# travistangvh/time-series-kafka-demo

Hardware: AMD Instinct MI355X
Metric: waveform_windows_per_sec (higher is better)
Workload: dtype bf16; 1 GPU; model=MyCNN5, global_batch=65536, seq_len=120, streams_per_gpu=65536, fs_hz=125, hipgraph=True, overlap=False, parallelism=dp1, mode=pipeline

## Files before the change

### tskd_amd/ops/csrc/preprocess_kernels.hip

```cpp

#include <hip/hip_runtime.h>
#include <cstdlib>
#include <math.h>

#include "tskd_common.h"

typedef __attribute__((ext_vector_type(4))) unsigned int u32x4_;
typedef __attribute__((ext_vector_type(4))) float f32x4_;

__device__ __forceinline__ long ring_head(const long long* dstate, long h) {
    return dstate ? (long)dstate[0] : h;
}
__device__ __forceinline__ long ring_nproc(const long long* dstate, long p) {
    return dstate ? (long)dstate[1] : p;
}

__global__ void advance_state_kernel(long long* dstate, int nb, int np) {
    if (threadIdx.x == 0 && blockIdx.x == 0) {
        dstate[0] += nb;
        dstate[1] += np;
    }
}

typedef float f32x2p_ __attribute__((ext_vector_type(2)));

#define ING_GRP 4
#define ING_GL 16
template <class DT>
__global__ void ingest_dense_kernel(
    const DT* __restrict__ raw,
    float* __restrict__ bsum,
    float* __restrict__ bcnt,
    const int* __restrict__ chan_map,
    int S, int CIN, int C, int T, int G,
    int bucket_len, long head_in,
    const long long* __restrict__ dstate, int BST)
{
    const long head = ring_head(dstate, head_in);
    const int head_mod = (int)(head % G);
    const int NB = T / bucket_len;
    const int NBG = (NB + ING_GRP - 1) / ING_GRP;
    const long nwaves = (long)S * CIN * NBG;
    const int wlane = threadIdx.x % WAVE;
    const int grp = wlane / ING_GL;
    const int lane = wlane % ING_GL;
    for (long w = (long)blockIdx.x * (blockDim.x / WAVE) + threadIdx.x / WAVE;
         w < nwaves; w += (long)gridDim.x * (blockDim.x / WAVE)) {
        const int wi = (int)w;
        const int bg = wi % NBG;
        const int wrem = wi / NBG;
        const int cin = wrem % CIN;
        const int s = wrem / CIN;
        const int b = bg * ING_GRP + grp;
        const bool active = b < NB;
        const DT* src = raw + ((long)s * CIN + cin) * T +
                        (long)(active ? b : 0) * bucket_len;
        float sum = 0.f, cnt = 0.f;
        if (active) {
            if constexpr (sizeof(DT) == 2) {
                const unsigned short* su = (const unsigned short*)src;
                const int mis = (int)(((size_t)su & 15) / 2);
                const u32x4_* vp = (const u32x4_*)(su - mis);
                const bool at_end = s == S - 1 && cin == CIN - 1 &&
                                    b == NB - 1;
                const int nch = (mis + bucket_len + (at_end ? 0 : 7)) / 8;
                for (int base = lane; base < nch; base += 5 * ING_GL) {
                    union { u32x4_ q; unsigned short h[8]; } v[5];
                    #pragma unroll
                    for (int u = 0; u < 5; ++u) {
                        const int pp = base + u * ING_GL;
                        v[u].q = __builtin_nontemporal_load(
                            &vp[pp < nch ? pp : 0]);
                    }
                    #pragma unroll
                    for (int u = 0; u < 5; ++u) {
                        const int pp = base + u * ING_GL;
                        if (pp >= nch) continue;
                        const int idx0 = pp * 8 - mis;
                        if (idx0 >= 0 && idx0 + 8 <= bucket_len) {
                            #pragma unroll
                            for (int j = 0; j < 8; ++j) {
                                const float f = bf16_to_f32(v[u].h[j]);
                                if (!isnan(f)) { sum += f; cnt += 1.f; }
                            }
                        } else {
                            #pragma unroll
                            for (int j = 0; j < 8; ++j) {
                                const unsigned k = (unsigned)(idx0 + j);
                                if (k < (unsigned)bucket_len) {
                                    const float f = bf16_to_f32(v[u].h[j]);
                                    if (!isnan(f)) { sum += f; cnt += 1.f; }
                                }
                            }
                        }
                    }
                }
                if (at_end)
                    for (int i = nch * 8 - mis + lane; i < bucket_len;
                         i += ING_GL) {
                        const float f = bf16_to_f32(su[i]);
                        if (!isnan(f)) { sum += f; cnt += 1.f; }
                    }
            } else {
                int pre = (int)(((16 - ((size_t)src & 15)) & 15) / 4);
                if (pre > bucket_len) pre = bucket_len;
                for (int i = lane; i < pre; i += ING_GL) {
                    const float f = (float)src[i];
                    if (!isnan(f)) { sum += f; cnt += 1.f; }
                }
                const int quad = (bucket_len - pre) / 4;
                const f32x4_* vp = (const f32x4_*)((const float*)src + pre);
                for (int base = lane; base < quad; base += 5 * ING_GL) {
                    f32x4_ v[5];
                    #pragma unroll
                    for (int u = 0; u < 5; ++u) {
                        const int pp = base + u * ING_GL;
                        v[u] = __builtin_nontemporal_load(
                            &vp[pp < quad ? pp : 0]);
                    }
                    #pragma unroll
                    for (int u = 0; u < 5; ++u) {
                        if (base + u * ING_GL < quad) {
                            if (!isnan(v[u].x)) { sum += v[u].x; cnt += 1.f; }
                            if (!isnan(v[u].y)) { sum += v[u].y; cnt += 1.f; }
                            if (!isnan(v[u].z)) { sum += v[u].z; cnt += 1.f; }
                            if (!isnan(v[u].w)) { sum += v[u].w; cnt += 1.f; }
                        }
                    }
                }
                for (int i = pre + quad * 4 + lane; i < bucket_len; i += ING_GL) {
                    const float f = (float)src[i];
                    if (!isnan(f)) { sum += f; cnt += 1.f; }
                }
            }
        }
        #pragma unroll
        for (int off = 8; off > 0; off >>= 1) {
            sum += __shfl_xor(sum, off);
            cnt += __shfl_xor(cnt, off);
        }
        if (lane == 0 && active) {
            const int c = chan_map[cin];
            int bi = head_mod + b;
            if (bi >= G) bi -= G;
            const long idx = (((long)s * C + c) * G + bi) * BST;
            bsum[idx] = sum;
            bcnt[idx] = cnt;
        }
    }
}

__global__ void ingest_events_kernel(
    const int* __restrict__ ev_stream, const int* __restrict__ ev_chan,
    const long* __restrict__ ev_bucket, const float* __restrict__ ev_val,
    float* __restrict__ bsum, float* __restrict__ bcnt,
    int C, int G, long n_events, long min_bucket, int BST)
{
    for (long i = (long)blockIdx.x * blockDim.x + threadIdx.x; i < n_events;
         i += (long)gridDim.x * blockDim.x) {
        const long b = ev_bucket[i];
        if (b < min_bucket) continue;
        const float v = ev_val[i];
        if (isnan(v)) continue;
        const long idx = (((long)ev_stream[i] * C + ev_chan[i]) * G
                          + b % G) * BST;
        atomicAdd(&bsum[idx], v);
        atomicAdd(&bcnt[idx], 1.f);
    }
}

__global__ void clear_buckets_kernel(
    float* __restrict__ bsum, float* __restrict__ bcnt,
    int S, int C, int G, long head, int nb, int BST)
{
    const long n = (long)S * C * nb;
    for (long i = (long)blockIdx.x * blockDim.x + threadIdx.x; i < n;
         i += (long)gridDim.x * blockDim.x) {
        const int j = (int)(i % nb);
        const long sc = i / nb;
        const long idx = (sc * G + (head + j) % G) * BST;
        bsum[idx] = 0.f;
        bcnt[idx] = 0.f;
    }
}

struct ResetRegions {
    float* base[3];
    int len[3];
    int vec[3];
    int units[3];
};

__global__ __launch_bounds__(256) void reset_streams_kernel(
    const int* __restrict__ sids, int n, ResetRegions rg,
    float* __restrict__ last_val, int S, int C)
{
    const int total = rg.units[0] + rg.units[1] + rg.units[2];
    const f32x4_ z4 = {0.f, 0.f, 0.f, 0.f};
    for (int k = blockIdx.y; k < n; k += gridDim.y) {
        const int s = sids[k];
        if ((unsigned)s >= (unsigned)S) continue;
        for (long u = (long)blockIdx.x * blockDim.x + threadIdx.x; u < total;
             u += (long)gridDim.x * blockDim.x) {
            float* base = rg.base[0];
            int len = rg.len[0], vec = rg.vec[0], v = (int)u;
            if (v >= rg.units[0]) {
                v -= rg.units[0];
                base = rg.base[1]; len = rg.len[1]; vec = rg.vec[1];
                if (v >= rg.units[1]) {
                    v -= rg.units[1];
                    base = rg.base[2]; len = rg.len[2]; vec = rg.vec[2];
                }
            }
            float* p = base + (long)s * len;
            if (vec) ((f32x4_*)p)[v] = z4;
            else p[v] = 0.f;
        }
        if (blockIdx.x == 0)
            for (int c = threadIdx.x; c < C; c += blockDim.x)
                last_val[(long)s * C + c] = NAN;
    }
}

template <bool RESTORE>
__global__ __launch_bounds__(256) void snapshot_streams_kernel(
    const int* __restrict__ sids, int n, float* bsum, float* bcnt,
    float* proc, float* last_val, int S, int C, int G, int BST,
    int b0, int p0, int nbk, int keep, float* rec_base)
{
    const int R = 2 * nbk + keep + 1;
    const long total = (long)C * R;
    for (int k = blockIdx.y; k < n; k += gridDim.y) {
        const int s = sids[k];
        if ((unsigned)s >= (unsigned)S) continue;
        float* rec = rec_base + (long)k * total;
        for (long u = (long)blockIdx.x * blockDim.x + threadIdx.x; u < total;
             u += (long)gridDim.x * blockDim.x) {
            const int c = (int)(u / R), r = (int)(u - (long)c * R);
            const long row = (long)s * C + c;
            float* p;
            if (r < 2 * nbk) {
                int g = b0 + (r >> 1);
                if (g >= G) g -= G;
                p = ((r & 1) ? bcnt : bsum) + (row * G + g) * BST;
            } else if (r < 2 * nbk + keep) {
                int g = p0 + (r - 2 * nbk);
                if (g >= G) g -= G;
                p = proc + row * G + g;
            } else {
                p = last_val + row;
            }
            if (RESTORE) *p = rec[u];
            else rec[u] = *p;
        }
    }
}

__global__ __launch_bounds__(256) void window_fill_kernel(
    const float* __restrict__ bsum, const float* __restrict__ bcnt,
    float* __restrict__ proc, float* __restrict__ last_val,
    int S, int C, int G, long phead_in, int np, int win_buckets,
    const long long* __restrict__ dstate, int BST)
{
    const long phead = ring_nproc(dstate, phead_in);
    constexpr int CHUNK = 64;
    const int MAXW = 64;
    __shared__ float lds_s[4][CHUNK + 64];
    __shared__ float lds_c[4][CHUNK + 64];
    __shared__ float lds_v[4][CHUNK];
    const int wave = threadIdx.x / WAVE;
    const int lane = threadIdx.x % WAVE;
    float* ls = lds_s[wave];
    float* lc = lds_c[wave];
    float* lv = lds_v[wave];
    (void)MAXW;

    const long nsc = (long)S * C;
    for (long sc = (long)blockIdx.x * 4 + wave; sc < nsc;
         sc += (long)gridDim.x * 4) {
        const float* bs = bsum + sc * G * BST;
        const float* bc = bcnt + sc * G * BST;
        float* pr = proc + sc * G;
        float carry = last_val[sc];
        int nan_prefix = 0;
        float first_val = NAN;

        for (int j0 = 0; j0 < np; j0 += CHUNK) {
            const int jn = min(CHUNK, np - j0);
            const int nload = jn + win_buckets - 1;
            for (int i = lane; i < nload; i += WAVE) {
                const long idx = (phead + j0 + i) % G;
                if (BST == 2) {
                    const f32x2p_ v = *(const f32x2p_*)(bs + idx * 2);
                    ls[i] = v.x;
                    lc[i] = v.y;
                } else {
                    ls[i] = bs[idx];
                    lc[i] = bc[idx];
                }
            }
            wave_sync();
            if (lane < jn) {
                float sum = 0.f, cnt = 0.f;
                for (int k = 0; k < win_buckets; ++k) {
                    sum += ls[lane + k];
                    cnt += lc[lane + k];
                }
                lv[lane] = (cnt > 0.f) ? sum / cnt : NAN;
            }
            wave_sync();
            if (lane == 0) {
                for (int j = 0; j < jn; ++j) {
                    const float v = lv[j];
                    if (isnan(v)) {
                        if (isnan(carry)) ++nan_prefix;
                        else lv[j] = carry;
                    } else {
                        if (isnan(carry)) first_val = v;
                        carry = v;
                    }
                }
            }
            wave_sync();
            if (lane < jn) pr[(phead + j0 + lane) % G] = lv[lane];
            wave_sync();
            carry = __shfl(carry, 0);
        }
        nan_prefix = __shfl(nan_prefix, 0);
        first_val = __shfl(first_val, 0);
        if (nan_prefix > 0) {
            const float fill = isnan(first_val) ? 0.f : first_val;
            for (int i = lane; i < nan_prefix; i += WAVE)
                pr[(phead + i) % G] = fill;
        }
        if (lane == 0) last_val[sc] = carry;
    }
}

template <class OT>
__global__ void window_gather_tlast2_kernel(
    const float* __restrict__ proc, OT* __restrict__ out,
    int S, int C, int G, int B, int WIN, int stride, long end_in,
    const long long* __restrict__ dstate, int end_extra)
{
    const long end = dstate ? (long)dstate[1] + end_extra : end_in;
    const long n = (long)S * B * WIN;
    for (long i = (long)blockIdx.x * blockDim.x + threadIdx.x; i < n;
         i += (long)gridDim.x * blockDim.x) {
        const int t = (int)(i % WIN);
        const int b = (int)((i / WIN) % B);
        const int s = (int)(i / ((long)WIN * B));
        const long wend = end - (long)(B - 1 - b) * stride;
        const long g = wend - WIN + t;
        const bool ok = g >= 0 && g < end && wend - WIN >= 0 && wend <= end;
        const int gi = ok ? (int)(g % G) : 0;
        const float* pr = proc + (long)s * C * G + gi;
        if constexpr (sizeof(OT) == 2) {
            unsigned int* od = (unsigned int*)(out + i * C);
            for (int c = 0; c < C; c += 2) {
                const unsigned int lo =
                    ok ? f32_to_bf16(pr[(long)c * G]) : 0u;
                const unsigned int hi =
                    ok ? f32_to_bf16(pr[(long)(c + 1) * G]) : 0u;
                od[c >> 1] = lo | (hi << 16);
            }
        } else {
            OT* od = out + i * C;
            for (int c = 0; c < C; ++c)
                od[c] = ok ? (OT)pr[(long)c * G] : (OT)0;
        }
    }
}

__global__ __launch_bounds__(256) void window_fill16_kernel(
    const float* __restrict__ bsum, const float* __restrict__ bcnt,
    float* __restrict__ proc, float* __restrict__ last_val,
    int S, int C, int G, long phead_in, int np, int win_buckets,
    const long long* __restrict__ dstate, int BST)
{
    const long phead = ring_nproc(dstate, phead_in);
    __shared__ float lds_v[4][64];
    const int wave = threadIdx.x / WAVE;
    const int lane = threadIdx.x % WAVE;
    const int grp = lane / 16, gl = lane % 16;
    float* lv = lds_v[wave] + grp * 16;

    const long nsc = (long)S * C;
    for (long sc0 = ((long)blockIdx.x * 4 + wave) * 4; sc0 < nsc;
         sc0 += (long)gridDim.x * 16) {
        const long sc = sc0 + grp;
        const bool live = sc < nsc;
        float carry = NAN, first_val = NAN, val = NAN;
        int nan_prefix = 0;
        if (live) {
            carry = last_val[sc];
            if (gl < np && BST == 2) {
                const f32x2p_* pk = (const f32x2p_*)(bsum + sc * G * 2);
                const int start = (int)((phead + gl) % G);
                const int first = min(win_buckets, G - start);
                const int rem = win_buckets - first;
                f32x2p_ a0 = {0.f, 0.f}, a1 = {0.f, 0.f};
                f32x2p_ a2 = {0.f, 0.f}, a3 = {0.f, 0.f};
                const f32x2p_* p1 = pk + start;
                int k = 0;
                for (; k + 4 <= first; k += 4) {
                    a0 += p1[k];     a1 += p1[k + 1];
                    a2 += p1[k + 2]; a3 += p1[k + 3];
                }
                for (; k < first; ++k) a0 += p1[k];
                int j = 0;
                for (; j + 4 <= rem; j += 4) {
                    a0 += pk[j];     a1 += pk[j + 1];
                    a2 += pk[j + 2]; a3 += pk[j + 3];
                }
                for (; j < rem; ++j) a0 += pk[j];
                const f32x2p_ t = (a0 + a1) + (a2 + a3);
                val = (t.y > 0.f) ? t.x / t.y : NAN;
            } else if (gl < np) {
                const float* bs = bsum + sc * G;
                const float* bc = bcnt + sc * G;
                const int start = (int)((phead + gl) % G);
                const int first = min(win_buckets, G - start);
                const int rem = win_buckets - first;
                float a0 = 0.f, a1 = 0.f, a2 = 0.f, a3 = 0.f;
                float c0 = 0.f, c1 = 0.f, c2 = 0.f, c3 = 0.f;
                const float* p1 = bs + start;
                const float* q1 = bc + start;
                int k = 0;
                for (; k + 4 <= first; k += 4) {
                    a0 += p1[k];     c0 += q1[k];
                    a1 += p1[k + 1]; c1 += q1[k + 1];
                    a2 += p1[k + 2]; c2 += q1[k + 2];
                    a3 += p1[k + 3]; c3 += q1[k + 3];
                }
                for (; k < first; ++k) { a0 += p1[k]; c0 += q1[k]; }
                int j = 0;
                for (; j + 4 <= rem; j += 4) {
                    a0 += bs[j];     c0 += bc[j];
                    a1 += bs[j + 1]; c1 += bc[j + 1];
                    a2 += bs[j + 2]; c2 += bc[j + 2];
                    a3 += bs[j + 3]; c3 += bc[j + 3];
                }
                for (; j < rem; ++j) { a0 += bs[j]; c0 += bc[j]; }
                const float sum = (a0 + a1) + (a2 + a3);
                const float cnt = (c0 + c1) + (c2 + c3);
                val = (cnt > 0.f) ? sum / cnt : NAN;
            }
        }
        lv[gl] = val;
        wave_sync();
        if (live && gl == 0) {
            for (int j = 0; j < np; ++j) {
                const float v = lv[j];
                if (isnan(v)) {
                    if (isnan(carry)) ++nan_prefix;
                    else lv[j] = carry;
                } else {
                    if (isnan(carry)) first_val = v;
                    carry = v;
                }
            }
            last_val[sc] = carry;
        }
        wave_sync();
        if (live && gl < np) {
            nan_prefix = __shfl(nan_prefix, grp * 16);
            first_val = __shfl(first_val, grp * 16);
            float outv = lv[gl];
            if (gl < nan_prefix)
                outv = isnan(first_val) ? 0.f : first_val;
            proc[sc * G + (phead + gl) % G] = outv;
        }
        wave_sync();
    }
}


template <class OT, bool TLAST = false>
__global__ void window_gather_kernel(
    const float* __restrict__ proc,
    OT* __restrict__ out,
    int S, int C, int G, int B, int WIN, int stride, long end_in,
    const long long* __restrict__ dstate, int end_extra)
{
    const long end = dstate ? (long)dstate[1] + end_extra : end_in;
    const int WQ = WIN / 4;
    const long n = (long)S * B * C * WQ;
    for (long i = (long)blockIdx.x * blockDim.x + threadIdx.x; i < n;
         i += (long)gridDim.x * blockDim.x) {
        const int tq = (int)(i % WQ);
        const int c = (int)((i / WQ) % C);
        const int b = (int)((i / ((long)WQ * C)) % B);
        const int s = (int)(i / ((long)WQ * C * B));
        const long wend = end - (long)(B - 1 - b) * stride;
        const long g0 = wend - WIN + tq * 4;
        const float* pr = proc + ((long)s * C + c) * G;
        float v[4];
        #pragma unroll
        for (int j = 0; j < 4; ++j) {
            const long g = g0 + j;
            v[j] = (g >= 0 && g < end && wend - WIN >= 0 && wend <= end)
                       ? pr[g % G] : 0.f;
        }
        if constexpr (TLAST) {
            const long ob = ((long)s * B + b) * C * WIN;
            #pragma unroll
            for (int j = 0; j < 4; ++j) {
                const long o = ob + (long)(tq * 4 + j) * C + c;
                if constexpr (sizeof(OT) == 2) out[o] = f32_to_bf16(v[j]);
                else out[o] = (OT)v[j];
            }
        } else {
            const long o = (((long)s * B + b) * C + c) * WIN + (long)tq * 4;
            if constexpr (sizeof(OT) == 2) {
                union { unsigned short h[4]; unsigned long long u; } pk;
                #pragma unroll
                for (int j = 0; j < 4; ++j) pk.h[j] = f32_to_bf16(v[j]);
                *(unsigned long long*)(out + o) = pk.u;
            } else {
                float4 pk = {v[0], v[1], v[2], v[3]};
                *(float4*)((float*)out + o) = pk;
            }
        }
    }
}

template <class OT>
__global__ void window_znorm_kernel(OT* __restrict__ w,
                                    long rows, int WIN, float eps)
{
    const int lane = threadIdx.x % WAVE;
    for (long r = (long)blockIdx.x * (blockDim.x / WAVE) + threadIdx.x / WAVE;
         r < rows; r += (long)gridDim.x * (blockDim.x / WAVE)) {
        OT* row = w + r * WIN;
        float sum = 0.f, sq = 0.f;
        for (int t = lane; t < WIN; t += WAVE) {
            float v;
            if constexpr (sizeof(OT) == 2) v = bf16_to_f32((unsigned short)row[t]);
            else v = (float)row[t];
            sum += v;
            sq = fmaf(v, v, sq);
        }
        #pragma unroll
        for (int off = 32; off > 0; off >>= 1) {
            sum += __shfl_xor(sum, off);
            sq += __shfl_xor(sq, off);
        }
        const float mean = sum / WIN;
        const float var = fmaxf(sq / WIN - mean * mean, 0.f);
        const float inv = 1.0f / fmaxf(sqrtf(var), eps);
        for (int t = lane; t < WIN; t += WAVE) {
            float v;
            if constexpr (sizeof(OT) == 2) v = bf16_to_f32((unsigned short)row[t]);
            else v = (float)row[t];
            v = (v - mean) * inv;
            if constexpr (sizeof(OT) == 2) row[t] = (OT)f32_to_bf16(v);
            else row[t] = (OT)v;
        }
    }
}

static inline int grid_for(long n, int block) {
    long g = (n + block - 1) / block;
    if (g > 16384) g = 16384;
    if (g < 1) g = 1;
    return (int)g;
}

extern "C" {

int tskd_preproc_ingest_dense(const void* raw, int raw_is_bf16,
                              float* bsum, float* bcnt, const int* chan_map,
                              int S, int CIN, int C, int T, int G,
                              int bucket_len, long head,
                              const long long* dstate, int bst,
                              void* stream) {
    hipStream_t st = (hipStream_t)stream;
    const int NB = T / bucket_len;
    if (NB <= 0 || S <= 0) return 0;
    const long nwaves = (long)S * CIN * ((NB + ING_GRP - 1) / ING_GRP);
    long cap = 32768;
    if (const char* gc = getenv("TSKD_INGEST_GRID")) cap = atol(gc);
    long blocks = (nwaves + 3) / 4;
    if (blocks > cap) blocks = cap;
    if (blocks < 1) blocks = 1;
    const int grid = (int)blocks;
    if (raw_is_bf16)
        hipLaunchKernelGGL((ingest_dense_kernel<unsigned short>), dim3(grid),
                           dim3(256), 0, st, (const unsigned short*)raw, bsum,
                           bcnt, chan_map, S, CIN, C, T, G, bucket_len, head,
                           dstate, bst);
    else
        hipLaunchKernelGGL((ingest_dense_kernel<float>), dim3(grid),
                           dim3(256), 0, st, (const float*)raw, bsum, bcnt,
                           chan_map, S, CIN, C, T, G, bucket_len, head, dstate,
                           bst);
    return (int)hipGetLastError();
}

int tskd_preproc_ingest_events(const int* ev_stream, const int* ev_chan,
                               const long* ev_bucket, const float* ev_val,
                               float* bsum, float* bcnt, int C, int G,
                               long n_events, long min_bucket, int bst,
                               void* stream) {
    if (n_events <= 0) return 0;
    hipLaunchKernelGGL(ingest_events_kernel, dim3(grid_for(n_events, 256)),
                       dim3(256), 0, (hipStream_t)stream, ev_stream, ev_chan,
                       ev_bucket, ev_val, bsum, bcnt, C, G, n_events,
                       min_bucket, bst);
    return (int)hipGetLastError();
}

int tskd_preproc_clear_buckets(float* bsum, float* bcnt, int S, int C, int G,
                               long head, int nb, int bst, void* stream) {
    if (nb <= 0) return 0;
    const long n = (long)S * C * nb;
    hipLaunchKernelGGL(clear_buckets_kernel, dim3(grid_for(n, 256)), dim3(256),
                       0, (hipStream_t)stream, bsum, bcnt, S, C, G, head, nb,
                       bst);
    return (int)hipGetLastError();
}

int tskd_preproc_reset_streams(const int* sids, int n, float* bsum,
                               float* bcnt, float* proc, float* last_val,
                               int S, int C, int G, int bst, void* stream) {
    if (n <= 0) return 0;
    const long cg = (long)C * G;
    if (S <= 0 || cg <= 0 || 3 * cg > 0x7fffffffL) return -4;
    if (bst == 2 && bcnt != bsum + 1) return -5;
    ResetRegions rg = {};
    int nreg = 0;
    auto add = [&](float* base, long len) {
        rg.base[nreg] = base;
        rg.len[nreg] = (int)len;
        rg.vec[nreg] = len % 4 == 0 && ((size_t)base & 15) == 0;
        rg.units[nreg] = (int)(rg.vec[nreg] ? len / 4 : len);
        ++nreg;
    };
    if (bst == 2) {
        add(bsum, 2 * cg);
    } else {
        add(bsum, cg);
        add(bcnt, cg);
    }
    add(proc, cg);
    const int total = rg.units[0] + rg.units[1] + rg.units[2];
    const int gy = n < 4096 ? n : 4096;
    int gx = (total + 255) / 256;
    if (gx > 4096 / gy) gx = 4096 / gy;
    if (gx < 1) gx = 1;
    hipLaunchKernelGGL(reset_streams_kernel, dim3(gx, gy), dim3(256), 0,
                       (hipStream_t)stream, sids, n, rg, last_val, S, C);
    return (int)hipGetLastError();
}

static int launch_snapshot(bool restore, const int* sids, int n, float* bsum,
                           float* bcnt, float* proc, float* last_val, int S,
                           int C, int G, int bst, long nproc, int nbk,
                           int keep, float* rec, hipStream_t st) {
    if (n <= 0) return 0;
    if (S <= 0 || C <= 0 || G <= 0 || nproc < 0) return -4;
    if (nbk < 0 || keep < 0 || nbk > G || keep > G || keep > nproc) return -4;
    if (bst != 1 && bst != 2) return -5;
    if (bst == 2 && bcnt != bsum + 1) return -5;
    const long total = (long)C * (2L * nbk + keep + 1);
    if (total > 0x7fffffffL) return -4;
    const int b0 = (int)(nproc % G), p0 = (int)((nproc - keep) % G);
    const int gy = n < 8192 ? n : 8192;
    long gx = (total + 255) / 256;
    if (gx > 8192 / gy) gx = 8192 / gy;
    if (gx < 1) gx = 1;
    if (restore)
        hipLaunchKernelGGL((snapshot_streams_kernel<true>), dim3((int)gx, gy),
                           dim3(256), 0, st, sids, n, bsum, bcnt, proc,
                           last_val, S, C, G, bst, b0, p0, nbk, keep, rec);
    else
        hipLaunchKernelGGL((snapshot_streams_kernel<false>),
                           dim3((int)gx, gy), dim3(256), 0, st, sids, n, bsum,
                           bcnt, proc, last_val, S, C, G, bst, b0, p0, nbk,
                           keep, rec);
    return (int)hipGetLastError();
}

int tskd_preproc_snapshot_streams(const int* sids, int n, const float* bsum,
                                  const float* bcnt, const float* proc,
                                  const float* last_val, int S, int C, int G,
                                  int bst, long nproc, int nbk, int keep,
                                  float* out, void* stream) {
    return launch_snapshot(false, sids, n, (float*)bsum, (float*)bcnt,
                           (float*)proc, (float*)last_val, S, C, G, bst,
                           nproc, nbk, keep, out, (hipStream_t)stream);
}

int tskd_preproc_restore_streams(const int* sids, int n, float* bsum,
                                 float* bcnt, float* proc, float* last_val,
                                 int S, int C, int G, int bst, long nproc,
                                 int nbk, int keep, const float* in,
                                 void* stream) {
    return launch_snapshot(true, sids, n, bsum, bcnt, proc, last_val, S, C, G,
                           bst, nproc, nbk, keep, (float*)in,
                           (hipStream_t)stream);
}

int tskd_preproc_window_fill(const float* bsum, const float* bcnt, float* proc,
                             float* last_val, int S, int C, int G, long phead,
                             int np, int win_buckets,
                             const long long* dstate, int bst, void* stream) {
    if (np <= 0) return 0;
    if (np <= 16) {
        const long nsc4 = ((long)S * C + 15) / 16;
        hipLaunchKernelGGL(window_fill16_kernel, dim3(grid_for(nsc4, 1)),
                           dim3(256), 0, (hipStream_t)stream, bsum, bcnt,
                           proc, last_val, S, C, G, phead, np, win_buckets,
                           dstate, bst);
        return (int)hipGetLastError();
    }
    const long nsc = (long)S * C * WAVE;
    hipLaunchKernelGGL(window_fill_kernel, dim3(grid_for(nsc, 256)), dim3(256),
                       0, (hipStream_t)stream, bsum, bcnt, proc, last_val, S,
                       C, G, phead, np, win_buckets, dstate, bst);
    return (int)hipGetLastError();
}

int tskd_preproc_advance_state(long long* dstate, int nb, int np,
                               void* stream) {
    hipLaunchKernelGGL(advance_state_kernel, dim3(1), dim3(64), 0,
                       (hipStream_t)stream, dstate, nb, np);
    return (int)hipGetLastError();
}

int tskd_preproc_window_gather(const float* proc, void* out, int out_is_bf16,
                               int out_timelast, int S, int C, int G, int B,
                               int WIN, int stride, long end,
                               const long long* dstate, int end_extra,
                               void* stream) {
    if (WIN % 4 != 0) return -3;
    const long n = (long)S * B * C * (WIN / 4);
    if (n <= 0) return 0;
    hipStream_t st = (hipStream_t)stream;
    const bool tlast2 = C % 2 == 0;
    const long n2 = (long)S * B * WIN;
    if (out_is_bf16) {
        if (out_timelast && tlast2)
            hipLaunchKernelGGL((window_gather_tlast2_kernel<unsigned short>),
                               dim3(grid_for(n2, 256)), dim3(256), 0, st,
                               proc, (unsigned short*)out, S, C, G, B, WIN,
                               stride, end, dstate, end_extra);
        else if (out_timelast)
            hipLaunchKernelGGL((window_gather_kernel<unsigned short, true>),
                               dim3(grid_for(n, 256)), dim3(256), 0, st, proc,
                               (unsigned short*)out, S, C, G, B, WIN, stride,
                               end, dstate, end_extra);
        else
            hipLaunchKernelGGL((window_gather_kernel<unsigned short>),
                               dim3(grid_for(n, 256)), dim3(256), 0, st, proc,
                               (unsigned short*)out, S, C, G, B, WIN, stride,
                               end, dstate, end_extra);
    } else {
        if (out_timelast && tlast2)
            hipLaunchKernelGGL((window_gather_tlast2_kernel<float>),
                               dim3(grid_for(n2, 256)), dim3(256), 0, st,
                               proc, (float*)out, S, C, G, B, WIN, stride,
                               end, dstate, end_extra);
        else if (out_timelast)
            hipLaunchKernelGGL((window_gather_kernel<float, true>),
                               dim3(grid_for(n, 256)), dim3(256), 0, st, proc,
                               (float*)out, S, C, G, B, WIN, stride, end,
                               dstate, end_extra);
        else
            hipLaunchKernelGGL((window_gather_kernel<float>),
                               dim3(grid_for(n, 256)), dim3(256), 0, st, proc,
                               (float*)out, S, C, G, B, WIN, stride, end,
                               dstate, end_extra);
    }
    return (int)hipGetLastError();
}

int tskd_preproc_window_znorm(void* w, int is_bf16, long rows, int win,
                              float eps, void* stream) {
    if (rows <= 0) return 0;
    const int grid = grid_for(rows * WAVE, 256);
    if (is_bf16)
        hipLaunchKernelGGL((window_znorm_kernel<unsigned short>), dim3(grid),
                           dim3(256), 0, (hipStream_t)stream,
                           (unsigned short*)w, rows, win, eps);
    else
        hipLaunchKernelGGL((window_znorm_kernel<float>), dim3(grid), dim3(256),
                           0, (hipStream_t)stream, (float*)w, rows, win, eps);
    return (int)hipGetLastError();
}

}
```

Measured before the change: 38.84 million windows/s.

## Stage bucket window into LDS with prefetch for small-step window fill

Adds a staged variant of the small-step window-fill kernel. Each 16-lane group loads the contiguous span of interleaved sum/count bucket pairs once into shared memory and prefetches the next stream-channel's data into registers while the current one computes. Window sums are then taken from LDS, fully unrolled for a compile-time window of 36 buckets, instead of re-reading global memory per output. The launcher selects this path by default when the bucket stride is 2 and the span fits 64 slots. This adds LDS use and template specialisation, and it can be turned off with an environment variable.

```diff
diff --git a/tskd_amd/ops/csrc/preprocess_kernels.hip b/tskd_amd/ops/csrc/preprocess_kernels.hip
--- a/tskd_amd/ops/csrc/preprocess_kernels.hip
+++ b/tskd_amd/ops/csrc/preprocess_kernels.hip
@@ -475,6 +475,123 @@
     }
 }
 
+#define F16_SLOTS 64
+#define F16_STRIDE 80
+template <int WB, int NQ>
+__global__ __launch_bounds__(256) void window_fill16_staged_kernel(
+    const float* __restrict__ bsum, float* __restrict__ proc,
+    float* __restrict__ last_val, int S, int C, int G, long phead_in, int np,
+    int win_buckets, const long long* __restrict__ dstate)
+{
+    static_assert(WB % 4 == 0 && WB + 15 <= F16_SLOTS, "");
+    static_assert(NQ >= 1 && NQ * 16 <= F16_SLOTS, "");
+    const long phead = ring_nproc(dstate, phead_in);
+    const int wb = WB ? WB : win_buckets;
+    __shared__ f32x2p_ lds_p[4][4][F16_STRIDE];
+    __shared__ float lds_v[4][64];
+    const int wave = threadIdx.x / WAVE;
+    const int lane = threadIdx.x % WAVE;
+    const int grp = lane / 16, gl = lane % 16;
+    float* lv = lds_v[wave] + grp * 16;
+    f32x2p_* row = lds_p[wave][grp];
+
+    const int s0 = (int)(phead % G);
+    const int span = np + wb - 1;
+    const bool nowrap = s0 + span <= G;
+    int eidx[NQ];
+    #pragma unroll
+    for (int q = 0; q < NQ; ++q) {
+        int e = s0 + gl + 16 * q;
+        if (e >= G) e -= G;
+        eidx[q] = gl + 16 * q < span ? e : 0;
+    }
+
+    const long nsc = (long)S * C;
+    const long stride = (long)gridDim.x * 16;
+    long sc0 = ((long)blockIdx.x * 4 + wave) * 4;
+    f32x2p_ ld[NQ];
+    float carry_ld = NAN;
+    auto fetch = [&](long base) {
+        const long sc = base + grp;
+        if (sc < nsc) {
+            const f32x2p_* pk = (const f32x2p_*)(bsum + sc * G * 2);
+            #pragma unroll
+            for (int q = 0; q < NQ; ++q) ld[q] = pk[eidx[q]];
+            carry_ld = last_val[sc];
+        }
+    };
+    if (sc0 < nsc) fetch(sc0);
+    for (; sc0 < nsc; sc0 += stride) {
+        const long sc = sc0 + grp;
+        const bool live = sc < nsc;
+        float carry = NAN, first_val = NAN, val = NAN;
+        int nan_prefix = 0;
+        if (live) {
+            carry = carry_ld;
+            #pragma unroll
+            for (int q = 0; q < NQ; ++q) row[gl + 16 * q] = ld[q];
+        }
+        if (sc0 + stride < nsc) fetch(sc0 + stride);
+        wave_sync();
+        if (live && gl < np) {
+            f32x2p_ a0 = {0.f, 0.f}, a1 = {0.f, 0.f};
+            f32x2p_ a2 = {0.f, 0.f}, a3 = {0.f, 0.f};
+            const f32x2p_* p1 = row + gl;
+            if (WB && nowrap) {
+                #pragma unroll
+                for (int k = 0; k < WB; k += 4) {
+                    a0 += p1[k];     a1 += p1[k + 1];
+                    a2 += p1[k + 2]; a3 += p1[k + 3];
+                }
+            } else {
+                const int start = (int)((phead + gl) % G);
+                const int first = min(wb, G - start);
+                const int rem = wb - first;
+                int k = 0;
+                for (; k + 4 <= first; k += 4) {
+                    a0 += p1[k];     a1 += p1[k + 1];
+                    a2 += p1[k + 2]; a3 += p1[k + 3];
+                }
+                for (; k < first; ++k) a0 += p1[k];
+                const f32x2p_* p2 = p1 + first;
+                int j = 0;
+                for (; j + 4 <= rem; j += 4) {
+                    a0 += p2[j];     a1 += p2[j + 1];
+                    a2 += p2[j + 2]; a3 += p2[j + 3];
+                }
+                for (; j < rem; ++j) a0 += p2[j];
+            }
+            const f32x2p_ t = (a0 + a1) + (a2 + a3);
+            val = (t.y > 0.f) ? t.x / t.y : NAN;
+        }
+        lv[gl] = val;
+        wave_sync();
+        if (live && gl == 0) {
+            for (int j = 0; j < np; ++j) {
+                const float v = lv[j];
+                if (isnan(v)) {
+                    if (isnan(carry)) ++nan_prefix;
+                    else lv[j] = carry;
+                } else {
+                    if (isnan(carry)) first_val = v;
+                    carry = v;
+                }
+            }
+            last_val[sc] = carry;
+        }
+        wave_sync();
+        if (live && gl < np) {
+            nan_prefix = __shfl(nan_prefix, grp * 16);
+            first_val = __shfl(first_val, grp * 16);
+            float outv = lv[gl];
+            if (gl < nan_prefix)
+                outv = isnan(first_val) ? 0.f : first_val;
+            proc[sc * G + (phead + gl) % G] = outv;
+        }
+        wave_sync();
+    }
+}
+
 
 template <class OT, bool TLAST = false>
 __global__ void window_gather_kernel(
@@ -709,6 +826,21 @@
     if (np <= 0) return 0;
     if (np <= 16) {
         const long nsc4 = ((long)S * C + 15) / 16;
+        const char* sk = getenv("TSKD_FILL16_STAGED");
+        const int span = np + win_buckets - 1;
+        if (bst == 2 && win_buckets >= 1 && span <= F16_SLOTS && span <= G &&
+            !(sk && atoi(sk) == 0)) {
+            const dim3 grid(grid_for(nsc4, 1));
+#define FILL16_STAGED(WB, NQ)                                                 \
+    hipLaunchKernelGGL((window_fill16_staged_kernel<WB, NQ>), grid,           \
+                       dim3(256), 0, (hipStream_t)stream, bsum, proc,         \
+                       last_val, S, C, G, phead, np, win_buckets, dstate)
+            if (win_buckets == 36 && span <= 48) FILL16_STAGED(36, 3);
+            else if (win_buckets == 36) FILL16_STAGED(36, 4);
+            else FILL16_STAGED(0, 4);
+#undef FILL16_STAGED
+            return (int)hipGetLastError();
+        }
         hipLaunchKernelGGL(window_fill16_kernel, dim3(grid_for(nsc4, 1)),
                            dim3(256), 0, (hipStream_t)stream, bsum, bcnt,
                            proc, last_val, S, C, G, phead, np, win_buckets,
```

After: 40.33 million windows/s, median of 6. 3.8% higher.
